# lixinustc/KVQ-Challenge-CVPR-NTIRE2024

Measured on AMD Instinct MI355X. Metric: videos/sec (8-frag x 32 x 224 x 224), higher is better.
Workload: dtype bf16

## Files before the change

include/kvq_hip.h:

```cpp
#ifndef KVQ_HIP_H
#define KVQ_HIP_H

#include <stddef.h>
#include <stdint.h>

#ifdef __cplusplus
extern "C" {
#endif

#define KVQ_ABI_VERSION 31
#define KVQ_MAX_STAGES 4

typedef enum { KVQ_DT_BF16 = 0, KVQ_DT_FP16 = 1 } KvqDtype;

typedef enum {
  KVQ_OK = 0,
  KVQ_ERR_NULL = -1,
  KVQ_ERR_SHAPE = -2,
  KVQ_ERR_UNSUPPORTED = -3,
  KVQ_ERR_WORKSPACE = -4,
  KVQ_ERR_HIP = -5
} KvqStatus;

int kvq_abi_version(void);
// ... 229 lines not shown
int kvq_block_tail(const KvqBlockTailArgs* host_args, void* stream);

int kvq_window_attention(const uint16_t* qkv, const int32_t* tok, const float* rpb, const float* fpb,
                         const float* bias_pack, int table_len, int center, int BW, int nW, int N, int num_heads, int use_mask,
                         int dtype, uint16_t* out, void* stream);

size_t kvq_attn_bias32_bytes(int n_types, int N, int num_heads);
int kvq_attn_bias32_build(const int32_t* tok, const float* rpb, const float* fpb, int table_len, int center,
                          int n_types, int N, int num_heads, int use_mask, void* out, float* max_abs, void* stream);
typedef struct {
  const uint16_t* qkv;
  const void* bias_dense;
  int32_t n_types, BW, nW, N, num_heads, dtype;
  uint16_t* out;
  const uint32_t* tile_skip;
  int32_t dsplit_from;
  const uint16_t* x_ln;
  const uint16_t* w_qkv;
  const float* b_qkv;
  float q_scale;
  const uint32_t* pad_mask;
} KvqAttnDenseArgs;
int kvq_window_attention32(const KvqAttnDenseArgs* host_args, void* stream);

int kvq_patch_im2col(const float* x, int B, int Cin, int T, int H, int W, int pd, int ph, int pw,
                     int dtype, uint16_t* out, void* stream);

int kvq_vqa_head(const float* feat, int B, int L, int C, int64_t stride_b, int64_t stride_l,
                 int64_t stride_c, const float* w1t, const float* w1, const float* b1, int hidden, const float* w2,
                 const float* b2, float* scratch, float* score, void* stream);

int kvq_vqa_head_classes(const float* feat, int B, int L, int C, int64_t stride_b, int64_t stride_l, int64_t stride_c,
                         const float* w1t, const float* b1, int hidden, const float* w2, const float* b2, int num_class,
                         int pre_pool, float* scratch, float* score, void* stream);

int kvq_simple_vqa_head(const float* feat, int B, int T, int Cin, const float* w1, const float* b1,
                        int hidden, const float* w2, const float* b2, float* scratch, float* score,
                        void* stream);

int kvq_fragment_gather(const void* video, int src_is_u8, int C, int T, int H, int W, const int32_t* hoff,
                        const int32_t* woff, int Fh, int Fw, int fs_h, int fs_w, int aligned,
                        const float* host_mean, const float* host_std, float* out, void* stream);
int kvq_fragment_gather_batch(const KvqFragmentSource* src, int C, int T, float* out, void* stream);

int kvq_resize_bilinear(const void* video, int src_is_u8, int C, int T, int H, int W, int rh, int rw, int cy,
                        int cx, int oh, int ow, int round_u8, const float* host_mean, const float* host_std,
// ... 139 lines not shown
```

kvq-challenge-cvpr-ntire2024_amd/_abi.py:

```python
from __future__ import annotations

import ctypes as C
import os
from typing import Optional

from . import _build

MAX_STAGES = 4
K_NAMES = ["im2col", "layernorm", "gemm_qkv", "attn", "gemm_proj", "gemm_fc1", "gemm_fc2", "gemm_merge",
           "gemm_embed", "tail", "embed", "merge"]
K_COUNT = len(K_NAMES)

EPI_BIAS_BF16, EPI_GELU_BF16, EPI_QKV_BF16, EPI_RESID_F32, EPI_STORE_F32, EPI_RELU_BF16, EPI_QGELU_BF16 = range(7)
DT_BF16, DT_FP16 = 0, 1
ABI_VERSION = 31


def dtype_code(dt) -> int:
    import torch
    is_int = isinstance(dt, int) and not isinstance(dt, bool)
    if (is_int and dt == DT_FP16) or (not is_int and dt in (torch.float16, "fp16", "float16")):
        return DT_FP16
    if (is_int and dt == DT_BF16) or (not is_int and dt in (torch.bfloat16, "bf16", "bfloat16")):
        return DT_BF16
# ... 13 lines not shown
                ("num_heads", C.c_int32 * MAX_STAGES), ("window", C.c_int32 * 3), ("mlp_ratio", C.c_int32),
                ("frag_bias", C.c_int32 * MAX_STAGES), ("adaptive_window", C.c_int32 * 3)]


class KvqSwinBlockW(C.Structure):
    _fields_ = [(n, p_void) for n in ("norm1_w", "norm1_b", "rpb_table", "fpb_table", "bias_pack", "qkv_w", "qkv_b", "proj_w",
                                      "proj_b", "norm2_w", "norm2_b", "fc1_w", "fc1_b", "fc2_w", "fc2_b", "tail_pack", "qkv_pack", "bias_dense")]


class KvqSwinMergeW(C.Structure):
    _fields_ = [(n, p_void) for n in ("norm_w", "norm_b", "red_w", "merge_pack")]


class KvqSwinWeights(C.Structure):
    _fields_ = [("embed_w", p_void), ("embed_b", p_void), ("embed_ln_w", p_void), ("embed_ln_b", p_void),
                ("embed_pack", p_void), ("blocks", C.POINTER(KvqSwinBlockW)), ("merges", KvqSwinMergeW * (MAX_STAGES - 1)),
                ("norm_w", p_void), ("norm_b", p_void)]


class KvqAttnDenseArgs(C.Structure):
    _fields_ = [("qkv", p_void), ("bias_dense", p_void), ("n_types", C.c_int32), ("BW", C.c_int32), ("nW", C.c_int32), ("N", C.c_int32),
                ("num_heads", C.c_int32), ("dtype", C.c_int32), ("out", p_void), ("tile_skip", p_void), ("dsplit_from", C.c_int32),
                ("x_ln", p_void), ("w_qkv", p_void), ("b_qkv", p_void), ("q_scale", C.c_float), ("pad_mask", p_void)]


class KvqGemmArgs(C.Structure):
    _fields_ = [("A", p_void), ("W", p_void), ("bias", p_void), ("M", C.c_int32), ("N", C.c_int32),
                ("K", C.c_int32), ("epilogue", C.c_int32), ("out_bf16", p_void), ("out_f32", p_void),
                ("num_heads", C.c_int32), ("q_scale", C.c_float), ("scatter_map", p_void),
                ("map_rows", C.c_int32), ("out_rows", C.c_int32), ("dtype", C.c_int32), ("resid_bf16", p_void), ("resid_f32", p_void),
                ("splitk_ws", p_void), ("splitk_ws_bytes", C.c_size_t), ("ldc", C.c_int32), ("col_off", C.c_int32),
                ("a_gather", p_void), ("a_rows", C.c_int32), ("a_phys_rows", C.c_int32)]


class KvqConvArgs(C.Structure):
    _fields_ = [("x", p_void), ("W", p_void), ("bias", p_void), ("taps", p_void), ("dims5", C.c_int32 * 5),
                ("kernel3", C.c_int32 * 3), ("stride3", C.c_int32 * 3), ("pad3", C.c_int32 * 3), ("Kpad", C.c_int32),
                ("N", C.c_int32), ("epilogue", C.c_int32), ("dtype", C.c_int32), ("out_bf16", p_void), ("out_f32", p_void),
                ("resid_bf16", p_void), ("resid_f32", p_void), ("splitk_ws", p_void), ("splitk_ws_bytes", C.c_size_t),
                ("ldc", C.c_int32), ("col_off", C.c_int32)]


class KvqNetTensor(C.Structure):
    _fields_ = [("B", C.c_int32), ("D", C.c_int32), ("H", C.c_int32), ("W", C.c_int32), ("C", C.c_int32), ("kind", C.c_int32)]


# ... 98 lines not shown
    "kvq_debug_gemm_trace": (i32, [p_void, i32]),
    "kvq_gemm_tile_mode": (i32, [i32]),
    "kvq_patch_embed_supported": (i32, [i32] * 8),
    "kvq_patch_embed_fragments_supported": (i32, [C.POINTER(KvqFragmentSource), i32, i32, i32, i32, i32, i32]),
    "kvq_patch_embed_pack_bytes": (sz, [i32, i32]),
    "kvq_patch_embed_pack": (i32, [p_void, p_void, p_void, p_void, i32, i32, p_void, p_void]),
    "kvq_patch_embed": (i32, [C.POINTER(KvqPatchEmbedArgs), p_void]),
    "kvq_patch_merge_supported": (i32, [i32]),
    "kvq_patch_merge_pack_bytes": (sz, [i32]),
    "kvq_patch_merge_pack": (i32, [p_void, p_void, p_void, i32, i32, p_void, p_void]),
    "kvq_patch_merge": (i32, [C.POINTER(KvqPatchMergeArgs), p_void]),
    "kvq_block_tail_supported": (i32, [i32, i32]),
    "kvq_block_tail_pack_bytes": (sz, [i32, i32]),
    "kvq_block_tail_pack": (i32, [p_void, p_void, p_void, p_void, p_void, p_void, p_void, p_void, i32, i32, p_void,
                                  p_void]),
    "kvq_block_tail_qkv_pack_bytes": (sz, [i32, i32]),
    "kvq_block_tail_qkv_pack": (i32, [p_void, i32, i32, p_void, p_void]),
    "kvq_block_tail": (i32, [C.POINTER(KvqBlockTailArgs), p_void]),
    "kvq_window_attention": (i32, [p_void, p_void, p_void, p_void, p_void, i32, i32, i32, i32, i32, i32, i32, i32, p_void,
                                   p_void]),
    "kvq_attn_bias32_bytes": (sz, [i32, i32, i32]),
    "kvq_attn_bias32_build": (i32, [p_void, p_void, p_void, i32, i32, i32, i32, i32, i32, p_void, p_void, p_void]),
    "kvq_window_attention32": (i32, [C.POINTER(KvqAttnDenseArgs), p_void]),
    "kvq_swin3d_bias_dense_bytes": (sz, [p_void, i32]),
    "kvq_swin3d_bias_dense_build": (i32, [p_void, i32, p_void, p_void, p_void, p_void, p_void]),
    "kvq_patch_im2col": (i32, [p_void, i32, i32, i32, i32, i32, i32, i32, i32, i32, p_void, p_void]),
    "kvq_vqa_head": (i32, [p_void, i32, i32, i32, i64, i64, i64, p_void, p_void, p_void, i32, p_void, p_void, p_void,
                           p_void, p_void]),
    "kvq_vqa_head_classes": (i32, [p_void, i32, i32, i32, i64, i64, i64, p_void, p_void, i32, p_void, p_void, i32, i32, p_void,
                                   p_void, p_void]),
    "kvq_simple_vqa_head": (i32, [p_void, i32, i32, i32, p_void, p_void, i32, p_void, p_void, p_void, p_void,
                                  p_void]),
    "kvq_resize_bilinear": (i32, [p_void, i32, i32, i32, i32, i32, i32, i32, i32, i32, i32, i32, i32, C.POINTER(f32),
                                  C.POINTER(f32), p_void, p_void]),
    "kvq_upsample_frames_out_dims": (i32, [i32, i32, C.c_double, C.POINTER(i32 * 2)]),
    "kvq_upsample_frames": (i32, [p_void, i32, i32, i32, i32, i32, C.c_double, p_void, p_void]),
    "kvq_im2col_nd": (i32, [p_void, i32, i32, C.POINTER(i64 * 5), C.POINTER(i32 * 5), C.POINTER(i32 * 3),
                            C.POINTER(i32 * 3), C.POINTER(i32 * 3), i32, p_void, p_void]),
    "kvq_pack_channels_last8": (i32, [p_void, C.POINTER(i32 * 5), C.POINTER(i64 * 5), i32, p_void, p_void]),
    "kvq_conv_stem_direct": (i32, [p_void, C.POINTER(i32 * 5), p_void, p_void, i32, C.POINTER(i32 * 3), C.POINTER(i32 * 3),
                                   C.POINTER(i32 * 3), i32, i32, p_void, p_void]),
    "kvq_pack_clip_cl4": (i32, [p_void, C.POINTER(i32 * 5), i32, i32, p_void, p_void]),
    "kvq_conv_stem_pool": (i32, [p_void, C.POINTER(i32 * 5), p_void, p_void, i32, i32, i32, p_void, p_void]),
    "kvq_conv_stem64_pool": (i32, [p_void, C.POINTER(i32 * 5), p_void, i32, p_void, p_void, i32, i32, p_void, i32, i32, p_void]),
    "kvq_slow_bottleneck_pack_bytes": (C.c_size_t, [i32, i32, i32]),
    "kvq_slow_bottleneck": (i32, [p_void, C.POINTER(i32 * 4), i32, i32, i32, p_void, i32, p_void, i32, p_void]),
# ... 76 lines not shown
```

kvq-challenge-cvpr-ntire2024_amd/csrc/attn32.hip:

```cpp
#include <stdlib.h>

#include "common.hpp"

#ifndef A32_ABL
#define A32_ABL 0
#endif
#ifndef A32_SUM
#define A32_SUM 0
#endif
#if (A32_ABL & 2)
#define A32_EXP(x) ((x) * 0.001f + 1.0f)
#else
#define A32_EXP(x) __builtin_amdgcn_exp2f(x)
#endif

#ifdef KVQ_DIAG
#define A32_DIAG_FLAG(x) (x)
#else
#define A32_DIAG_FLAG(x) false
#endif

namespace kvq {

constexpr int A32_KB = 13;
// ... 196 lines not shown
  }
  ls += ls1;
  if (A32_SUM == 1) ls = (lv0[0] + lv0[1]) + (lv1[0] + lv1[1]);
  ls = a32_pair_sum(ls);
  a32_finish<E>(O, ls, orow, store);
#undef A32_NR
}

struct Attn32Params {
  const uint16_t* qkv;
  const u32x4* image;
  int BW, nW, N, nH, n_types, qsplit;
  uint16_t* out;
  const uint32_t* tile_skip;
  int dsplit_from;
  const uint16_t* x_ln;
  const uint16_t* w_qkv;
  const float* b_qkv;
  float q_scale;
  uint16_t* q_out;
  const uint32_t* pad_mask;
  bool no_q_store;
  bool image_one;
};

template <typename E, int KS>
__device__ __forceinline__ void a32_fused_qkv(const Attn32Params& p, unsigned char* slot, int bw, int h, int N) {
  using V8 = typename E::v8;
  const int tid = threadIdx.x, lane = tid & 63, j = lane & 15, g = lane >> 4;
  const int wave = __builtin_amdgcn_readfirstlane(tid >> 6);
  const int C = KS * 32;
  const size_t Mtot = (size_t)p.BW * N;
  const uint16_t* xw = p.x_ln + (size_t)bw * N * C;
  uint16_t* qo = p.q_out + ((size_t)h * Mtot + (size_t)bw * N) * 32;
  V8 wf[6][KS];
  float bias[6][4];
#pragma unroll
  for (int c = 0; c < 6; ++c) {
    const int which = c >> 1, half = c & 1, frow = which * C + h * 32 + half * 16;
#pragma unroll
    for (int ks = 0; ks < KS; ++ks) wf[c][ks] = *reinterpret_cast<const V8*>(p.w_qkv + (size_t)(frow + j) * C + 32 * ks + 8 * g);
    const f32x4 b4 = *reinterpret_cast<const f32x4*>(p.b_qkv + frow + 4 * g);
#pragma unroll
    for (int r = 0; r < 4; ++r) bias[c][r] = b4[r];
  }
  const int nrt = (N + 15) / 16;
  V8 xn[KS];
  {
    const int rowc = min(16 * wave + j, N - 1);
#pragma unroll
    for (int ks = 0; ks < KS; ++ks) xn[ks] = *reinterpret_cast<const V8*>(xw + (size_t)rowc * C + 32 * ks + 8 * g);
  }
#pragma unroll 1
  for (int rt = wave; rt < nrt; rt += A32_WAVES) {
    const int row = 16 * rt + j;
    V8 xf[KS];
#pragma unroll
    for (int ks = 0; ks < KS; ++ks) xf[ks] = xn[ks];
    if (rt + A32_WAVES < nrt) {
      const int rowc = min(row + 16 * A32_WAVES, N - 1);
#pragma unroll
      for (int ks = 0; ks < KS; ++ks) xn[ks] = *reinterpret_cast<const V8*>(xw + (size_t)rowc * C + 32 * ks + 8 * g);
    }
#pragma unroll
    for (int c = 0; c < 6; ++c) {
      const int which = c >> 1, half = c & 1;
      f32x4 acc = {0.f, 0.f, 0.f, 0.f};
#pragma unroll
      for (int ks = 0; ks < KS; ++ks) acc = E::mfma16(wf[c][ks], xf[ks], acc);
      const float sc = which == 0 ? p.q_scale : 1.f;
      const u32x2 v = {E::pack2((acc[0] + bias[c][0]) * sc, (acc[1] + bias[c][1]) * sc),
                       E::pack2((acc[2] + bias[c][2]) * sc, (acc[3] + bias[c][3]) * sc)};
      if (row < N) {
        if (which == 0) {
          if (!A32_DIAG_FLAG(p.no_q_store)) *reinterpret_cast<u32x2*>(qo + (size_t)row * 32 + half * 16 + 4 * g) = v;
        } else if (which == 1) {
          *reinterpret_cast<u32x2*>(slot + row * 64 + (((2 * half + (g >> 1)) ^ ((row >> 2) & 3)) << 4) + (g & 1) * 8) = v;
        } else {
          *reinterpret_cast<u32x2*>(slot + A32_K_BYTES + row * 64 + (16 * half + 4 * g) * 2) = v;
        }
      }
    }
  }
}

template <typename E, bool FUSED, bool DSPLIT, bool SHORT = false>
__global__ __launch_bounds__(A32_WAVES * 64, 3) __attribute__((amdgpu_waves_per_eu(3, 3))) void window_attention32_kernel(Attn32Params p) {
  fp16_saturate_mode();
  extern __shared__ __attribute__((aligned(16))) unsigned char smem[];
  int* ticket = reinterpret_cast<int*>(smem + A32_OFF_CTR);
  using V8 = typename E::v8;
  const int nclip = p.BW / p.nW, nrep = p.nW / p.n_types, npair = p.n_types * p.nH, per_pair = nclip * nrep * p.qsplit;
  const int xcd = blockIdx.x & 7, slot_i = blockIdx.x >> 3;
  int pair, clip, rep, part;
  if (FUSED) {
    const int per_type = p.nH * nclip * nrep, wt_ = (slot_i / per_type) * 8 + xcd, sub = slot_i % per_type;
    if (wt_ >= p.n_types) return;
    const int h_ = sub % p.nH, rest = sub / p.nH;
    pair = wt_ * p.nH + h_; clip = rest % nclip; rep = rest / nclip; part = 0;
  } else {
    const int sub = slot_i % per_pair;
    pair = (slot_i / per_pair) * 8 + xcd;
    clip = sub % nclip; rep = (sub / nclip) % nrep; part = sub / (nclip * nrep);
  }
  if (pair >= npair) return;
  const int wt = pair / p.nH, h = pair - wt * p.nH, w = rep * p.n_types + wt, bw = clip * p.nW + w;
  const int tid = threadIdx.x, lane = tid & 63, N = p.N, nqb = (N + 31) >> 5;
  const int wave = __builtin_amdgcn_readfirstlane(tid >> 6);
  const size_t Mtot = (size_t)p.BW * N;
  const int C = p.nH * 32;
  const uint16_t* Qg = p.qkv + ((size_t)h * Mtot + (size_t)bw * N) * 32;

  if (tid < 64) *reinterpret_cast<u32x4*>(smem + A32_OFF_ZERO + tid * 16) = (u32x4){0u, 0u, 0u, 0u};
  if (FUSED) {
    for (int i = tid; i < (A32_ROWS - N) * 8; i += A32_WAVES * 64)
      *reinterpret_cast<u32x4*>(smem + (i & 4 ? A32_K_BYTES : 0) + (N + (i >> 3)) * 64 + (i & 3) * 16) = (u32x4){0u, 0u, 0u, 0u};
    a32_fused_qkv<E, 3>(p, smem, bw, h, N);
  } else {
    const uint16_t* Kg = p.qkv + ((size_t)(1 * p.nH + h) * Mtot + (size_t)bw * N) * 32;
    const uint16_t* Vg = p.qkv + ((size_t)(2 * p.nH + h) * Mtot + (size_t)bw * N) * 32;
    const __amdgpu_buffer_rsrc_t rk = __builtin_amdgcn_make_buffer_rsrc(const_cast<uint16_t*>(Kg), 0, N * 64, 0x00020000);
    const __amdgpu_buffer_rsrc_t rv = __builtin_amdgcn_make_buffer_rsrc(const_cast<uint16_t*>(Vg), 0, N * 64, 0x00020000);
    const unsigned vo_k = (unsigned)(lane >> 2) * 64u + (unsigned)((lane & 3) ^ ((lane >> 4) & 3)) * 16u, vo_v = (unsigned)lane * 16u;
    for (int it = wave; it < A32_ROWS / 16; it += A32_WAVES) {
      __builtin_amdgcn_raw_ptr_buffer_load_lds(rk, (a32_lds_t)(smem + it * 1024), 16, vo_k, it * 1024, 0, 0);
      __builtin_amdgcn_raw_ptr_buffer_load_lds(rv, (a32_lds_t)(smem + A32_K_BYTES + it * 1024), 16, vo_v, it * 1024, 0, 0);
    }
  }
  const int q_lo = part * nqb / p.qsplit, q_hi = (part + 1) * nqb / p.qsplit;
  if (tid == 0) *ticket = q_lo;
  asm volatile("s_waitcnt vmcnt(0)" ::: "memory");
  __syncthreads();
  if (!FUSED && p.pad_mask) {
    const uint32_t* pm = p.pad_mask + (size_t)w * A32_KB;
    const int c = tid & 3;
    const float* kb = p.b_qkv + C + h * 32 + 8 * c;
    const float* vb = p.b_qkv + 2 * C + h * 32 + 8 * c;
    const u32x4 kc = {E::pack2(kb[0], kb[1]), E::pack2(kb[2], kb[3]), E::pack2(kb[4], kb[5]), E::pack2(kb[6], kb[7])};
    const u32x4 vc = {E::pack2(vb[0], vb[1]), E::pack2(vb[2], vb[3]), E::pack2(vb[4], vb[5]), E::pack2(vb[6], vb[7])};
    for (int r = tid >> 2; r < N; r += A32_WAVES * 16)
// ... 106 lines not shown
    const int half = tile & 1, blk = tile >> 1, qb = blk / A32_KB, kb = blk - qb * A32_KB, qq = 32 * qb + ql;
    const int2 tq = tokL[qq < N ? qq : N - 1];
    const float shift = rmax[qq < N ? qq : N - 1];
    float v[8];
#pragma unroll
    for (int e = 0; e < 8; ++e) {
      const int r = 8 * half + e, key = 32 * kb + (r & 3) + 8 * (r >> 2) + 4 * hi;
      float b = 0.f;
      if (key >= N) {
        b = A32_OFF;
      } else if (qq < N) {
        bool masked;
        b = value(tq, key, &masked);
        if (masked) b = -100.0f;
        b -= shift;
      }
      v[e] = b;
    }
    *reinterpret_cast<u32x4*>(img + (size_t)tile * 512 + lane * 8) =
        (u32x4){Fp16::pack2_raw(v[0], v[1]), Fp16::pack2_raw(v[2], v[3]), Fp16::pack2_raw(v[4], v[5]), Fp16::pack2_raw(v[6], v[7])};
  }
}

template <typename E, bool FUSED, bool DSPLIT, bool SHORT>
static int launch_attn32_form(const Attn32Params& p, hipStream_t st) {
  auto kern = window_attention32_kernel<E, FUSED, DSPLIT, SHORT>;
  LdsOptIn opt;
  if (int rc = opt.ensure(reinterpret_cast<const void*>(kern), A32_LDS)) return rc;
  const int nclip = p.BW / p.nW, nrep = p.nW / p.n_types, npair = p.n_types * p.nH;
  unsigned grid = (unsigned)(8 * ceil_div(npair, 8) * nclip * nrep * p.qsplit);
  if (FUSED) grid = (unsigned)(8 * ceil_div(p.n_types, 8) * p.nH * nclip * nrep);
  hipLaunchKernelGGL(kern, dim3(grid), dim3(A32_WAVES * 64), A32_LDS, st, p);
  KVQ_CHECK_LAUNCH("window_attention32_kernel");
  return KVQ_OK;
}

template <typename E, bool FUSED, bool DSPLIT>
static int launch_attn32(const Attn32Params& p, hipStream_t st) {
  return p.N > 384 && p.N <= 392 ? launch_attn32_form<E, FUSED, DSPLIT, true>(p, st) : launch_attn32_form<E, FUSED, DSPLIT, false>(p, st);
}

template <typename E>
static int launch_attn32_e(const Attn32Params& p, hipStream_t st) {
  if (p.x_ln) return p.dsplit_from >= 0 ? launch_attn32<E, true, true>(p, st) : launch_attn32<E, true, false>(p, st);
  return p.dsplit_from >= 0 ? launch_attn32<E, false, true>(p, st) : launch_attn32<E, false, false>(p, st);
}

}

extern "C" size_t kvq_attn_bias32_bytes(int n_types, int N, int num_heads) {
  if (n_types <= 0 || N < 1 || N > 400 || num_heads <= 0) return 0;
  return (size_t)n_types * num_heads * ((N + 31) / 32) * kvq::A32_KB * 2048 + 2048;
}

extern "C" int kvq_attn_bias32_build(const int32_t* tok, const float* rpb, const float* fpb, int table_len, int center,
                                          int nW, int N, int num_heads, int use_mask, void* out, float* max_abs, void* stream) {
  using namespace kvq;
  KVQ_REQUIRE(tok && rpb && out, KVQ_ERR_NULL, "kvq_attn_bias32_build: NULL pointer");
  KVQ_REQUIRE(kvq_attn_bias32_bytes(nW, N, num_heads) > 0 && table_len > 0, KVQ_ERR_SHAPE,
              "kvq_attn_bias32_build: bad shape nW=%d N=%d nH=%d", nW, N, num_heads);
  KVQ_REQUIRE(((size_t)out & 15) == 0, KVQ_ERR_SHAPE, "kvq_attn_bias32_build: out must be 16-byte aligned");
  Bias32BuildParams p{tok, rpb, fpb, table_len, center, nW, N, num_heads, use_mask, (uint16_t*)out, (unsigned*)max_abs};
  const size_t lds = (size_t)table_len * 8 + (size_t)N * 12;
  KVQ_REQUIRE(lds <= 64 * 1024, KVQ_ERR_UNSUPPORTED, "kvq_attn_bias32_build: table of %d entries does not fit the builder's LDS", table_len);
  hipLaunchKernelGGL(bias32_build_kernel, dim3((unsigned)num_heads, (unsigned)nW), dim3(256), lds, (hipStream_t)stream, p);
  KVQ_CHECK_LAUNCH("bias32_build_kernel");
  return KVQ_OK;
}

extern "C" int kvq_window_attention32(const KvqAttnDenseArgs* a, void* stream) {
  using namespace kvq;
  KVQ_REQUIRE(a && a->qkv && a->bias_dense && a->out, KVQ_ERR_NULL, "kvq_window_attention32: NULL pointer");
  const int BW = a->BW, nW = a->nW, N = a->N, num_heads = a->num_heads, n_types = a->n_types;
  KVQ_REQUIRE(BW > 0 && nW > 0 && BW % nW == 0 && num_heads > 0 && n_types > 0 && nW % n_types == 0, KVQ_ERR_SHAPE,
              "kvq_window_attention32: bad shape BW=%d nW=%d n_types=%d nH=%d", BW, nW, n_types, num_heads);
  KVQ_REQUIRE(N >= 1 && N <= 400, KVQ_ERR_UNSUPPORTED, "kvq_window_attention32: window of %d tokens unsupported (1..400)", N);
  KVQ_REQUIRE(((size_t)a->bias_dense & 15) == 0, KVQ_ERR_SHAPE, "kvq_window_attention32: the bias image must be 16-byte aligned");
  KVQ_REQUIRE(a->dtype == KVQ_DT_BF16 || a->dtype == KVQ_DT_FP16, KVQ_ERR_UNSUPPORTED, "kvq_window_attention32: dtype %d", a->dtype);
  KVQ_REQUIRE(a->dsplit_from < 0 || (N == 392 && a->dsplit_from < nW), KVQ_ERR_UNSUPPORTED,
              "kvq_window_attention32: depth-split windows need the (8,7,7) window (N = 392); got N=%d from=%d", N, a->dsplit_from);
  const int units = BW * num_heads, nqb = (N + 31) / 32;
  int qsplit = units >= 768 ? 1 : 768 / units;
  const int qsplit_max = latency_mode() ? 4 : 1;
  qsplit = qsplit > qsplit_max ? qsplit_max : qsplit;
  qsplit = qsplit > nqb ? nqb : qsplit;
  Attn32Params p{a->qkv, (const u32x4*)a->bias_dense, BW, nW, N, num_heads, n_types, qsplit, a->out, a->tile_skip,
                     a->dsplit_from < 0 ? -1 : a->dsplit_from};
#ifdef KVQ_DIAG
  { static const bool one = getenv("KVQ_IMAGE_ONE_TYPE") && atoi(getenv("KVQ_IMAGE_ONE_TYPE")) == 1; p.image_one = one; }
  { static const bool nq = getenv("KVQ_NO_Q_STORE") && atoi(getenv("KVQ_NO_Q_STORE")) == 1; p.no_q_store = nq; }
#endif
  if (a->pad_mask) {
    KVQ_REQUIRE(a->b_qkv && !a->x_ln, KVQ_ERR_NULL, "kvq_window_attention32: pad_mask needs b_qkv (and excludes the fused projection)");
    p.pad_mask = a->pad_mask; p.b_qkv = a->b_qkv;
  }
  if (a->x_ln) {
    const int C = 32 * num_heads;
    KVQ_REQUIRE(a->w_qkv && a->b_qkv, KVQ_ERR_NULL, "kvq_window_attention32: x_ln without w_qkv / b_qkv");
    KVQ_REQUIRE(C == 96, KVQ_ERR_UNSUPPORTED, "kvq_window_attention32: the fused qkv projection is built for C = 96 (got %d)", C);
    KVQ_REQUIRE((((size_t)a->x_ln | (size_t)a->w_qkv | (size_t)a->b_qkv) & 15) == 0, KVQ_ERR_SHAPE,
                "kvq_window_attention32: x_ln / w_qkv / b_qkv must be 16-byte aligned");
    p.qsplit = 1;
    p.x_ln = a->x_ln; p.w_qkv = a->w_qkv; p.b_qkv = a->b_qkv; p.q_scale = a->q_scale; p.q_out = const_cast<uint16_t*>(a->qkv);
  }
  hipStream_t st = (hipStream_t)stream;
  return a->dtype == KVQ_DT_FP16 ? launch_attn32_e<Fp16>(p, st) : launch_attn32_e<Bf16>(p, st);
}
```

kvq-challenge-cvpr-ntire2024_amd/csrc/plan.hip:

```cpp
#include <math.h>
#include <stdlib.h>
#include <string.h>

#include <vector>

#include "common.hpp"
#include "tail.hpp"

#ifdef KVQ_DIAG
static int skip_mask() {
  static const int m = [] {
    const int v = getenv("KVQ_SKIP") ? atoi(getenv("KVQ_SKIP")) : 0;
    if (v) fprintf(stderr, "libkvq_hip (KVQ_DIAG build): KVQ_SKIP=%d leaves launch families out - scores are GARBAGE, timing only\n", v);
    return v;
  }();
  return m;
}
#else
static constexpr int skip_mask() { return 0; }
#endif

namespace kvq {

struct StageGeom {
// ... 425 lines not shown
  const bool embed_fused = w->embed_pack && kvq_patch_embed_supported(cfg.in_chans, cfg.patch[0], cfg.patch[1], cfg.patch[2], cfg.embed_dim, pl->T, pl->H, pl->W);
  auto fused_tail = [&](int i, int bk) -> bool { return w->blocks[bk].tail_pack && kvq_block_tail_supported(pl->st[i].C, cfg.mlp_ratio * pl->st[i].C); };
  auto attn_fuses_qkv = [&](int i, int bk) -> bool {
    const StageGeom& g = pl->st[i];
    const KvqSwinBlockW& bw = w->blocks[bk];
    return bw.bias_dense && bw.qkv_b && g.Lp == g.L && g.C == 96 && g.N <= 400;
  };
  bool x16[KVQ_MAX_STAGES] = {false, false, false, false};
  if (resid16_on && !any_tap) {
    int blk0 = 0;
    for (int i = 0; i < cfg.num_stages - 1 && i <= stage_hi; blk0 += pl->st[i].depth, ++i) {
      if (i < stage_lo) continue;
      const StageGeom& g = pl->st[i];
      const bool produced16 = i == 0 ? (stage_lo == 0 && embed_fused) : (i > stage_lo && (fused_merge(i - 1) || pl->dtype == KVQ_DT_FP16));
      bool ok = produced16;
      for (int b = 0; ok && b < g.depth; ++b) {
        const KvqSwinBlockW& bw = w->blocks[blk0 + b];
        const int par = (b & 1) && g.shifted_any ? 1 : 0;
        ok = fused_tail(i, blk0 + b) && bw.norm1_w && bw.norm1_b && g.d_dst[par];
      }
      x16[i] = ok;
    }
  }
  bool x16_cur = false;
  auto f32_only = [&](const char* what) -> int {
    KVQ_REQUIRE(!x16_cur, KVQ_ERR_UNSUPPORTED, "kvq_swin3d_forward: internal: %s on an fp16 residual stream", what);
    return KVQ_OK;
  };

  const int L0 = pl->D0 * pl->H0 * pl->W0, E = cfg.embed_dim;
  float* cur = xa;
  float* oth = xb;
  bool first_ln1_ready = false;
  if (stage_lo > 0) {
    const StageGeom& g0 = pl->st[stage_lo];
    KVQ_CHECK_HIP(hipMemcpyAsync(xa, io, (size_t)B * g0.L * g0.C * sizeof(float), hipMemcpyDeviceToDevice, st));
  } else if (embed_fused) {
    KvqPatchEmbedArgs ea{};
    ea.x = x; ea.frag = frag; ea.B = B; ea.in_chans = cfg.in_chans; ea.T = pl->T; ea.H = pl->H; ea.W = pl->W;
    ea.pd = cfg.patch[0]; ea.ph = cfg.patch[1]; ea.pw = cfg.patch[2]; ea.embed_dim = E; ea.pack = w->embed_pack;
    ea.has_norm = w->embed_ln_w ? 1 : 0; ea.out = xa; ea.eps = 1e-5f; ea.dtype = pl->dtype; ea.out_f16 = x16[0] ? 1 : 0;
    x16_cur = x16[0];
    const StageGeom& g0 = pl->st[0];
    if (g0.Lp == g0.L && g0.d_dst[0] && w->blocks[0].norm1_w && w->blocks[0].norm1_b) {
      ea.next_norm_w = w->blocks[0].norm1_w; ea.next_norm_b = w->blocks[0].norm1_b; ea.next_dst = g0.d_dst[0];
      ea.next_ln = bln; ea.next_rows = g0.Lp;
// ... 25 lines not shown
    KVQ_CHECK_HIP(hipMemcpyAsync(pl->taps[idx], cur, elems * sizeof(float), hipMemcpyDeviceToDevice, st));
    return KVQ_OK;
  };
  if (stage_lo == 0) KVQ_TRY(tap(0, (size_t)B * L0 * E));

  int blk = 0;
  for (int i = 0; i < stage_lo; ++i) blk += pl->st[i].depth;
  size_t out_elems = 0;
  bool merged_ln1_ready = false;
  for (int i = stage_lo; i <= stage_hi; ++i) {
    const StageGeom& g = pl->st[i];
    const int C = g.C, M = B * g.Lp, ML = B * g.L;
    bool ln1_ready = (i == 0 && first_ln1_ready) || merged_ln1_ready;
    bool qkv_ready = false;
    merged_ln1_ready = false;
    if (i == stage_lo && i > 0) cur = xa, oth = xb;
    for (int b = 0; b < g.depth; ++b, ++blk) {
      const KvqSwinBlockW& bw = w->blocks[blk];
      KVQ_REQUIRE(bw.norm1_w && bw.rpb_table && bw.qkv_w && bw.proj_w && bw.fc1_w && bw.fc2_w, KVQ_ERR_NULL,
                  "kvq_swin3d_forward: block %d weights incomplete", blk);
      const int par = (b & 1) && g.shifted_any ? 1 : 0;
      const bool fuse_qkv = attn_fuses_qkv(i, blk);
      const float qs = bw.bias_dense ? kQScaleLog2 : kQScale;
      if (g.Lp != g.L && bw.qkv_b && qkv_ready) {
      } else if (g.Lp != g.L && bw.qkv_b) {
        if (!ln1_ready) KVQ_TRY(ln(pl, st, cur, nullptr, 1, g.L, g.L, C, bw.norm1_w, bw.norm1_b, bln, nullptr, x16_cur));
        KVQ_TRY(gemm(pl, st, KVQ_K_GEMM_QKV, bln, bw.qkv_w, bw.qkv_b, ML, 3 * C, C, KVQ_EPI_QKV_BF16, bbig, nullptr, g.nH,
                     qs, g.d_dst[par], g.L, g.Lp));
        if (!(bw.bias_dense && g.d_padmask[par]))
          KVQ_TRY(kvq_qkv_fill_pad(bbig, bw.qkv_b, g.d_pad[par], g.Lp - g.L, B, g.Lp, g.nH, qs, pl->dtype, st));
      } else if (!qkv_ready) {
        if (!ln1_ready) KVQ_TRY(ln(pl, st, cur, g.d_src[par], 1, g.L, g.Lp, C, bw.norm1_w, bw.norm1_b, bln, nullptr, x16_cur));
        if (!fuse_qkv)
          KVQ_TRY_UNLESS(8 | (i == cfg.num_stages - 1 ? 32 : 0), gemm(pl, st, KVQ_K_GEMM_QKV, bln, bw.qkv_w, bw.qkv_b, M, 3 * C, C, KVQ_EPI_QKV_BF16, bbig, nullptr, g.nH, qs));
      }
      ln1_ready = false;
      qkv_ready = false;
      if (bw.bias_dense) {
        Bracket br(pl, st, KVQ_K_ATTN, 4 + par, 4.0 * M * g.N * C + (fuse_qkv ? 6.0 * M * C * C : 0.0),
                   (fuse_qkv ? 2.0 * 2.0 * M * C + 6.0 * C * C : 2.0 * 4.0 * M * C) + (double)kvq_swin3d_bias_dense_bytes(pl, blk));
        KvqAttnDenseArgs aa{};
        aa.qkv = bbig; aa.bias_dense = bw.bias_dense; aa.n_types = bias_types(g, par); aa.BW = B * g.nW; aa.nW = g.nW; aa.N = g.N;
        aa.num_heads = g.nH; aa.dtype = pl->dtype; aa.out = bo; aa.tile_skip = (const uint32_t*)g.d_skip[par];
        const int slabs = g.Dp / g.ws[0];
        aa.dsplit_from = (par == 1 && g.N == 392 && g.ws[0] == 8 && g.ws[1] == 7 && g.ws[2] == 7 && g.ss[0] == 4 && slabs >= 1)
                             ? g.nW - g.nW / slabs : -1;
        if (fuse_qkv) { aa.x_ln = bln; aa.w_qkv = bw.qkv_w; aa.b_qkv = bw.qkv_b; aa.q_scale = qs; }
        if (g.Lp != g.L && bw.qkv_b && g.d_padmask[par]) { aa.pad_mask = (const uint32_t*)g.d_padmask[par]; aa.b_qkv = bw.qkv_b; }
        KVQ_TRY_UNLESS(1 | (i == cfg.num_stages - 1 ? 32 : 0), kvq_window_attention32(&aa, st));
      } else {
        Bracket br(pl, st, KVQ_K_ATTN, (cfg.frag_bias[i] ? 2 : 0) + par, 4.0 * M * g.N * C, 2.0 * 4.0 * M * C);
        KVQ_TRY(kvq_window_attention(bbig, g.d_tok[par], bw.rpb_table, cfg.frag_bias[i] ? bw.fpb_table : nullptr,
                                     bw.bias_pack,
                                     pl->table_len, pl->center, B * g.nW, g.nW, g.N, g.nH, par, pl->dtype, bo,
                                     st));
      }
      const int hidden = cfg.mlp_ratio * C;
      if (fused_tail(i, blk)) {
        KvqBlockTailArgs ta{};
        ta.attn = bo; ta.x = cur; ta.scatter_map = g.d_src[par]; ta.map_rows = g.Lp; ta.out_rows = g.L;
        ta.M = M; ta.C = C; ta.hidden = hidden; ta.pack = bw.tail_pack; ta.eps = 1e-5f; ta.dtype = pl->dtype;
        ta.x_f16 = x16_cur ? 1 : 0;
        const int npar = ((b + 1) & 1) && g.shifted_any ? 1 : 0;
        if (g.Lp != g.L) ta.attn_gather = g.d_dst[par];
        const bool padded_qkv = g.Lp != g.L && b + 1 < g.depth && g.d_dst[npar] && g.d_padmask[npar] && w->blocks[blk + 1].bias_dense;
        const int32_t* nmap = (g.Lp == g.L || padded_qkv) ? g.d_dst[npar] : nullptr;
        if (b + 1 < g.depth && nmap) {
          const KvqSwinBlockW& nb = w->blocks[blk + 1];
          KVQ_REQUIRE(nb.norm1_w && nb.norm1_b, KVQ_ERR_NULL, "kvq_swin3d_forward: block %d norm1 missing", blk + 1);
          ta.next_norm_w = nb.norm1_w; ta.next_norm_b = nb.norm1_b; ta.next_dst = nmap;
          ta.next_rows = g.Lp;
          if (!attn_fuses_qkv(i, blk + 1) && nb.qkv_pack && nb.qkv_b && nb.bias_dense && (g.Lp == g.L || padded_qkv) && kvq_block_tail_qkv_pack_bytes(C, hidden) > 0) {
            ta.next_qkv_pack = nb.qkv_pack; ta.next_qkv_b = nb.qkv_b; ta.qkv_out = bbig; ta.q_scale = kQScaleLog2; ta.num_heads = g.nH;
            qkv_ready = true;
          } else if (g.Lp == g.L) {
            ta.next_ln = bln;
            ln1_ready = true;
          } else {
            ta.next_norm_w = nullptr; ta.next_norm_b = nullptr; ta.next_dst = nullptr; ta.next_rows = 0;
          }
        }
        Bracket br(pl, st, KVQ_K_TAIL, kvq::tailmm_geometry_code(C, hidden) * 1000 + (C / 32) * 10 + (ln1_ready ? 1 : 0) + (qkv_ready ? 2 : 0), 2.0 * M * C * C + 4.0 * (double)ML * C * hidden + (qkv_ready ? 6.0 * M * C * C : 0.0),
                   (double)M * C * 2.0 + (double)ML * C * ((x16_cur ? 4.0 : 8.0) + (ln1_ready ? 2.0 : 0.0) + (qkv_ready ? 6.0 : 0.0)));
        KVQ_TRY_UNLESS(C <= 192 ? 2 : 4, kvq_block_tail(&ta, st));
        continue;
      }
      KVQ_TRY(f32_only("the proj / MLP GEMM chain"));
      if (g.Lp != g.L) {
        KvqGemmArgs pa{};
        pa.A = bo; pa.W = bw.proj_w; pa.bias = bw.proj_b; pa.M = ML; pa.N = C; pa.K = C; pa.epilogue = KVQ_EPI_RESID_F32; pa.out_f32 = cur;
        pa.dtype = pl->dtype; pa.a_gather = g.d_dst[par]; pa.a_rows = g.L; pa.a_phys_rows = g.Lp;
        Bracket br(pl, st, KVQ_K_GEMM_PROJ, gemm_variant(ML, C, C) * 10 + KVQ_EPI_RESID_F32, 2.0 * M * C * C,
                   2.0 * ((double)ML * C + (double)C * C) + 8.0 * ML * C);
        KVQ_TRY(kvq_gemm_bf16(&pa, st));
      } else {
        KVQ_TRY_UNLESS(i == cfg.num_stages - 1 ? 32 : 0, gemm(pl, st, KVQ_K_GEMM_PROJ, bo, bw.proj_w, bw.proj_b, M, C, C, KVQ_EPI_RESID_F32, nullptr, cur, 0, 1.f,
                     g.d_src[par], g.Lp, g.L));
// ... 74 lines not shown
```

kvq-challenge-cvpr-ntire2024_amd/kernels.py:

```python
from __future__ import annotations

import ctypes as C
from typing import Optional, Sequence

import torch

from . import _abi
from ._abi import check, current_stream, dtype_code, lib, ptr, stream_of

HALF_TYPES = (torch.float16, torch.bfloat16)


def _need_gpu(*ts):
    for t in ts:
        if t is not None and not t.is_cuda:
            raise _abi.KvqError("kvq_amd kernels need tensors on a HIP device (no CPU fallback exists)")


def device_name() -> str:
    buf = C.create_string_buffer(256)
    check(lib().kvq_device_name(buf, 256), "kvq_device_name")
    return buf.value.decode()


# ... 79 lines not shown
    check(lib().kvq_window_attention(ptr(qkv), ptr(tok), ptr(rpb), ptr(fpb), ptr(bias_pack), rpb.shape[0], center, BW, nW, N, nH,
                                     int(use_mask), dtype_code(qkv.dtype), ptr(out), current_stream()),
          "kvq_window_attention")
    return out


LOG2E = 1.4426950408889634


def attn_bias32(tok: torch.Tensor, rpb: torch.Tensor, fpb: Optional[torch.Tensor], center: int, nW: int, N: int, use_mask: bool):
    _need_gpu(tok, rpb, fpb)
    nH = rpb.shape[1]
    out = torch.empty(lib().kvq_attn_bias32_bytes(nW, N, nH), dtype=torch.uint8, device=rpb.device)
    big = torch.zeros(1, dtype=torch.float32, device=rpb.device)
    check(lib().kvq_attn_bias32_build(ptr(tok), ptr(rpb), ptr(fpb), rpb.shape[0], center, nW, N, nH, int(use_mask),
                                      ptr(out), ptr(big), current_stream()), "kvq_attn_bias32_build")
    out.max_abs_bias = big
    return out


def window_attention32(qkv: torch.Tensor, image: torch.Tensor, nW: int, N: int, n_types: Optional[int] = None,
                       tile_skip: Optional[torch.Tensor] = None, out: Optional[torch.Tensor] = None, dsplit_from: int = -1,
                       x_ln: Optional[torch.Tensor] = None, w_qkv: Optional[torch.Tensor] = None, b_qkv: Optional[torch.Tensor] = None,
                       q_scale: float = 1.0, pad_mask: Optional[torch.Tensor] = None):
    _need_gpu(qkv, image, tile_skip, out, pad_mask)
    assert qkv.dtype in HALF_TYPES and qkv.is_contiguous()
    nH = qkv.shape[1]
    BW = qkv.shape[2] // N
    if out is None:
        out = torch.empty(BW * N, nH * 32, dtype=qkv.dtype, device=qkv.device)
    a = _abi.KvqAttnDenseArgs()
    a.qkv, a.bias_dense, a.n_types, a.BW, a.nW, a.N, a.num_heads = ptr(qkv), ptr(image), nW if n_types is None else n_types, BW, nW, N, nH
    a.dtype, a.out, a.tile_skip, a.dsplit_from = dtype_code(qkv.dtype), ptr(out), ptr(tile_skip), dsplit_from
    if x_ln is not None:
        _need_gpu(x_ln, w_qkv, b_qkv)
        assert x_ln.dtype == qkv.dtype == w_qkv.dtype and x_ln.is_contiguous() and w_qkv.is_contiguous() and b_qkv.dtype == torch.float32
        a.x_ln, a.w_qkv, a.b_qkv, a.q_scale = ptr(x_ln), ptr(w_qkv), ptr(b_qkv), q_scale
    if pad_mask is not None:
        _need_gpu(b_qkv)
        assert pad_mask.dtype == torch.int32 and pad_mask.is_contiguous() and (b_qkv is None or b_qkv.dtype == torch.float32)
        a.pad_mask, a.b_qkv = ptr(pad_mask), ptr(b_qkv)
    check(lib().kvq_window_attention32(C.byref(a), current_stream()), "kvq_window_attention32")
    return out


def patch_im2col(x: torch.Tensor, patch: Sequence[int], out_dtype=torch.float16):
    _need_gpu(x)
    assert x.dtype == torch.float32 and x.is_contiguous()
    B, Cin, T, H, W = x.shape
    pd, ph, pw = patch
    D, Hh, Ww = -(-T // pd), -(-H // ph), -(-W // pw)
    out = torch.empty(B * D * Hh * Ww, Cin * pd * ph * pw, dtype=out_dtype, device=x.device)
    check(lib().kvq_patch_im2col(ptr(x), B, Cin, T, H, W, pd, ph, pw, dtype_code(out_dtype), ptr(out),
                                 current_stream()), "kvq_patch_im2col")
    return out


def vqa_head(feat: torch.Tensor, w1, b1, w2, b2, w1t=None):
    _need_gpu(feat, w1, b1, w2, b2, w1t)
    assert feat.dtype == torch.float32 and feat.dim() == 5
    B, Cc, D, H, W = feat.shape
    L = D * H * W
    sb, sc, sd, sh, sw = feat.stride()
    if not (sh == W * sw and sd == H * sh):
# ... 727 lines not shown
```

Measured before the change: 364.7.

## Fuse norm1 LayerNorm and window gather into fused-QKV attention kernel

Adds a NORM variant of the fused-QKV window attention kernel. It reads the fp16 residual stream directly through the window map, applies LayerNorm with gamma and beta staged in LDS, and then runs the QKV projection. The planner uses it when it is eligible, skipping the separate LN launch and the LN that the previous block tail produced, which removes a write and read of the normalized activations. The cost is more per-row work and extra LDS inside the attention kernel, plus gathered, non-contiguous row loads.

After: 366.1 (median of 6 runs). About the same (+0.4%).

```diff
diff --git a/include/kvq_hip.h b/include/kvq_hip.h
--- a/include/kvq_hip.h
+++ b/include/kvq_hip.h
@@ -275,6 +275,15 @@
   const uint32_t* pad_mask;
 } KvqAttnDenseArgs;
 int kvq_window_attention32(const KvqAttnDenseArgs* host_args, void* stream);
+typedef struct KvqAttnNorm1Args {
+  const void* x;
+  const int32_t* window_map;
+  int L;
+  const float* norm1_w;
+  const float* norm1_b;
+  float eps;
+} KvqAttnNorm1Args;
+int kvq_window_attention32_norm1(const KvqAttnDenseArgs* host_args, const KvqAttnNorm1Args* norm, void* stream);
 
 int kvq_patch_im2col(const float* x, int B, int Cin, int T, int H, int W, int pd, int ph, int pw,
                      int dtype, uint16_t* out, void* stream);
diff --git a/kvq-challenge-cvpr-ntire2024_amd/_abi.py b/kvq-challenge-cvpr-ntire2024_amd/_abi.py
--- a/kvq-challenge-cvpr-ntire2024_amd/_abi.py
+++ b/kvq-challenge-cvpr-ntire2024_amd/_abi.py
@@ -59,6 +59,10 @@
     _fields_ = [("qkv", p_void), ("bias_dense", p_void), ("n_types", C.c_int32), ("BW", C.c_int32), ("nW", C.c_int32), ("N", C.c_int32),
                 ("num_heads", C.c_int32), ("dtype", C.c_int32), ("out", p_void), ("tile_skip", p_void), ("dsplit_from", C.c_int32),
                 ("x_ln", p_void), ("w_qkv", p_void), ("b_qkv", p_void), ("q_scale", C.c_float), ("pad_mask", p_void)]
+
+
+class KvqAttnNorm1Args(C.Structure):
+    _fields_ = [("x", p_void), ("window_map", p_void), ("L", C.c_int32), ("norm1_w", p_void), ("norm1_b", p_void), ("eps", C.c_float)]
 
 
 class KvqGemmArgs(C.Structure):
@@ -203,6 +207,7 @@
     "kvq_attn_bias32_bytes": (sz, [i32, i32, i32]),
     "kvq_attn_bias32_build": (i32, [p_void, p_void, p_void, i32, i32, i32, i32, i32, i32, p_void, p_void, p_void]),
     "kvq_window_attention32": (i32, [C.POINTER(KvqAttnDenseArgs), p_void]),
+    "kvq_window_attention32_norm1": (i32, [C.POINTER(KvqAttnDenseArgs), C.POINTER(KvqAttnNorm1Args), p_void]),
     "kvq_swin3d_bias_dense_bytes": (sz, [p_void, i32]),
     "kvq_swin3d_bias_dense_build": (i32, [p_void, i32, p_void, p_void, p_void, p_void, p_void]),
     "kvq_patch_im2col": (i32, [p_void, i32, i32, i32, i32, i32, i32, i32, i32, i32, p_void, p_void]),
diff --git a/kvq-challenge-cvpr-ntire2024_amd/csrc/attn32.hip b/kvq-challenge-cvpr-ntire2024_amd/csrc/attn32.hip
--- a/kvq-challenge-cvpr-ntire2024_amd/csrc/attn32.hip
+++ b/kvq-challenge-cvpr-ntire2024_amd/csrc/attn32.hip
@@ -242,16 +242,29 @@
   const uint32_t* pad_mask;
   bool no_q_store;
   bool image_one;
+  const uint16_t* x16;
+  const int32_t* map;
+  int L;
+  const float* n1w;
+  const float* n1b;
+  float eps;
 };
-
-template <typename E, int KS>
+constexpr int A32_OFF_NRM = A32_LDS;
+constexpr int A32_LDS_NORM = A32_OFF_NRM + 2 * 96 * 4;
+
+template <typename E, int KS, bool NORM = false>
 __device__ __forceinline__ void a32_fused_qkv(const Attn32Params& p, unsigned char* slot, int bw, int h, int N) {
   using V8 = typename E::v8;
   const int tid = threadIdx.x, lane = tid & 63, j = lane & 15, g = lane >> 4;
   const int wave = __builtin_amdgcn_readfirstlane(tid >> 6);
   const int C = KS * 32;
   const size_t Mtot = (size_t)p.BW * N;
-  const uint16_t* xw = p.x_ln + (size_t)bw * N * C;
+  const uint16_t* xw = NORM ? nullptr : p.x_ln + (size_t)bw * N * C;
+  const int clip = NORM ? bw / p.nW : 0, wl = NORM ? bw - clip * p.nW : 0;
+  auto rowp = [&](int r) __attribute__((always_inline)) -> const uint16_t* {
+    if constexpr (NORM) return p.x16 + ((size_t)clip * p.L + p.map[(size_t)wl * N + r]) * C;
+    else return xw + (size_t)r * C;
+  };
   uint16_t* qo = p.q_out + ((size_t)h * Mtot + (size_t)bw * N) * 32;
   V8 wf[6][KS];
   float bias[6][4];
@@ -269,7 +282,7 @@
   {
     const int rowc = min(16 * wave + j, N - 1);
 #pragma unroll
-    for (int ks = 0; ks < KS; ++ks) xn[ks] = *reinterpret_cast<const V8*>(xw + (size_t)rowc * C + 32 * ks + 8 * g);
+    for (int ks = 0; ks < KS; ++ks) xn[ks] = *reinterpret_cast<const V8*>(rowp(rowc) + 32 * ks + 8 * g);
   }
 #pragma unroll 1
   for (int rt = wave; rt < nrt; rt += A32_WAVES) {
@@ -280,7 +293,46 @@
     if (rt + A32_WAVES < nrt) {
       const int rowc = min(row + 16 * A32_WAVES, N - 1);
 #pragma unroll
-      for (int ks = 0; ks < KS; ++ks) xn[ks] = *reinterpret_cast<const V8*>(xw + (size_t)rowc * C + 32 * ks + 8 * g);
+      for (int ks = 0; ks < KS; ++ks) xn[ks] = *reinterpret_cast<const V8*>(rowp(rowc) + 32 * ks + 8 * g);
+    }
+    if constexpr (NORM) {
+      typedef __attribute__((ext_vector_type(8))) _Float16 h8;
+      const float* nrm = reinterpret_cast<const float*>(slot + A32_OFF_NRM);
+      float s = 0.f;
+#pragma unroll
+      for (int ks = 0; ks < KS; ++ks) {
+        const h8 v = __builtin_bit_cast(h8, xf[ks]);
+        s += ((float)v[0] + (float)v[1]) + ((float)v[2] + (float)v[3]) + (((float)v[4] + (float)v[5]) + ((float)v[6] + (float)v[7]));
+      }
+      s += __shfl_xor(s, 16);
+      s += __shfl_xor(s, 32);
+      const float mean = s / (float)C;
+      float sq = 0.f;
+#pragma unroll
+      for (int ks = 0; ks < KS; ++ks) {
+        const h8 v = __builtin_bit_cast(h8, xf[ks]);
+#pragma unroll
+        for (int e = 0; e < 8; ++e) {
+          const float d = (float)v[e] - mean;
+          sq += d * d;
+        }
+      }
+      sq += __shfl_xor(sq, 16);
+      sq += __shfl_xor(sq, 32);
+      const float rstd = rsqrtf(sq / (float)C + p.eps), nmr = -mean * rstd;
+#pragma unroll
+      for (int ks = 0; ks < KS; ++ks) {
+        const h8 v = __builtin_bit_cast(h8, xf[ks]);
+        const f32x4 g0 = *reinterpret_cast<const f32x4*>(nrm + 32 * ks + 8 * g), g1 = *reinterpret_cast<const f32x4*>(nrm + 32 * ks + 8 * g + 4);
+        const f32x4 b0 = *reinterpret_cast<const f32x4*>(nrm + C + 32 * ks + 8 * g), b1 = *reinterpret_cast<const f32x4*>(nrm + C + 32 * ks + 8 * g + 4);
+        float y[8];
+#pragma unroll
+        for (int e = 0; e < 4; ++e) {
+          y[e] = fmaf(fmaf((float)v[e], rstd, nmr), g0[e], b0[e]);
+          y[4 + e] = fmaf(fmaf((float)v[4 + e], rstd, nmr), g1[e], b1[e]);
+        }
+        xf[ks] = __builtin_bit_cast(V8, (u32x4){E::pack2(y[0], y[1]), E::pack2(y[2], y[3]), E::pack2(y[4], y[5]), E::pack2(y[6], y[7])});
+      }
     }
 #pragma unroll
     for (int c = 0; c < 6; ++c) {
@@ -304,7 +356,7 @@
   }
 }
 
-template <typename E, bool FUSED, bool DSPLIT, bool SHORT = false>
+template <typename E, bool FUSED, bool DSPLIT, bool SHORT = false, bool NORM = false>
 __global__ __launch_bounds__(A32_WAVES * 64, 3) __attribute__((amdgpu_waves_per_eu(3, 3))) void window_attention32_kernel(Attn32Params p) {
   fp16_saturate_mode();
   extern __shared__ __attribute__((aligned(16))) unsigned char smem[];
@@ -335,7 +387,11 @@
   if (FUSED) {
     for (int i = tid; i < (A32_ROWS - N) * 8; i += A32_WAVES * 64)
       *reinterpret_cast<u32x4*>(smem + (i & 4 ? A32_K_BYTES : 0) + (N + (i >> 3)) * 64 + (i & 3) * 16) = (u32x4){0u, 0u, 0u, 0u};
-    a32_fused_qkv<E, 3>(p, smem, bw, h, N);
+    if constexpr (NORM) {
+      if (tid < 2 * 96) reinterpret_cast<float*>(smem + A32_OFF_NRM)[tid] = tid < 96 ? p.n1w[tid] : p.n1b[tid - 96];
+      __syncthreads();
+    }
+    a32_fused_qkv<E, 3, NORM>(p, smem, bw, h, N);
   } else {
     const uint16_t* Kg = p.qkv + ((size_t)(1 * p.nH + h) * Mtot + (size_t)bw * N) * 32;
     const uint16_t* Vg = p.qkv + ((size_t)(2 * p.nH + h) * Mtot + (size_t)bw * N) * 32;
@@ -488,15 +544,16 @@
   }
 }
 
-template <typename E, bool FUSED, bool DSPLIT, bool SHORT>
+template <typename E, bool FUSED, bool DSPLIT, bool SHORT, bool NORM = false>
 static int launch_attn32_form(const Attn32Params& p, hipStream_t st) {
-  auto kern = window_attention32_kernel<E, FUSED, DSPLIT, SHORT>;
+  auto kern = window_attention32_kernel<E, FUSED, DSPLIT, SHORT, NORM>;
+  constexpr int lds = NORM ? A32_LDS_NORM : A32_LDS;
   LdsOptIn opt;
-  if (int rc = opt.ensure(reinterpret_cast<const void*>(kern), A32_LDS)) return rc;
+  if (int rc = opt.ensure(reinterpret_cast<const void*>(kern), lds)) return rc;
   const int nclip = p.BW / p.nW, nrep = p.nW / p.n_types, npair = p.n_types * p.nH;
   unsigned grid = (unsigned)(8 * ceil_div(npair, 8) * nclip * nrep * p.qsplit);
   if (FUSED) grid = (unsigned)(8 * ceil_div(p.n_types, 8) * p.nH * nclip * nrep);
-  hipLaunchKernelGGL(kern, dim3(grid), dim3(A32_WAVES * 64), A32_LDS, st, p);
+  hipLaunchKernelGGL(kern, dim3(grid), dim3(A32_WAVES * 64), lds, st, p);
   KVQ_CHECK_LAUNCH("window_attention32_kernel");
   return KVQ_OK;
 }
@@ -506,8 +563,14 @@
   return p.N > 384 && p.N <= 392 ? launch_attn32_form<E, FUSED, DSPLIT, true>(p, st) : launch_attn32_form<E, FUSED, DSPLIT, false>(p, st);
 }
 
+template <typename E, bool DSPLIT>
+static int launch_attn32_norm(const Attn32Params& p, hipStream_t st) {
+  return p.N > 384 && p.N <= 392 ? launch_attn32_form<E, true, DSPLIT, true, true>(p, st) : launch_attn32_form<E, true, DSPLIT, false, true>(p, st);
+}
+
 template <typename E>
 static int launch_attn32_e(const Attn32Params& p, hipStream_t st) {
+  if (p.x16) return p.dsplit_from >= 0 ? launch_attn32_norm<E, true>(p, st) : launch_attn32_norm<E, false>(p, st);
   if (p.x_ln) return p.dsplit_from >= 0 ? launch_attn32<E, true, true>(p, st) : launch_attn32<E, true, false>(p, st);
   return p.dsplit_from >= 0 ? launch_attn32<E, false, true>(p, st) : launch_attn32<E, false, false>(p, st);
 }
@@ -534,7 +597,7 @@
   return KVQ_OK;
 }
 
-extern "C" int kvq_window_attention32(const KvqAttnDenseArgs* a, void* stream) {
+static int attn32_entry(const KvqAttnDenseArgs* a, const KvqAttnNorm1Args* n, void* stream) {
   using namespace kvq;
   KVQ_REQUIRE(a && a->qkv && a->bias_dense && a->out, KVQ_ERR_NULL, "kvq_window_attention32: NULL pointer");
   const int BW = a->BW, nW = a->nW, N = a->N, num_heads = a->num_heads, n_types = a->n_types;
@@ -560,15 +623,29 @@
     KVQ_REQUIRE(a->b_qkv && !a->x_ln, KVQ_ERR_NULL, "kvq_window_attention32: pad_mask needs b_qkv (and excludes the fused projection)");
     p.pad_mask = a->pad_mask; p.b_qkv = a->b_qkv;
   }
-  if (a->x_ln) {
+  if (n) {
+    KVQ_REQUIRE(n->x && n->window_map && n->norm1_w && n->norm1_b && !a->x_ln && !a->pad_mask, KVQ_ERR_NULL,
+                "kvq_window_attention32_norm1: NULL pointer, or x_ln / pad_mask given");
+    KVQ_REQUIRE(n->L == nW * N, KVQ_ERR_SHAPE, "kvq_window_attention32_norm1: un-padded partitions only (L=%d, nW=%d, N=%d)", n->L, nW, N);
+    KVQ_REQUIRE(((size_t)n->x & 15) == 0, KVQ_ERR_SHAPE, "kvq_window_attention32_norm1: x must be 16-byte aligned");
+    p.x16 = (const uint16_t*)n->x; p.map = n->window_map; p.L = n->L; p.n1w = n->norm1_w; p.n1b = n->norm1_b; p.eps = n->eps;
+  }
+  if (a->x_ln || n) {
     const int C = 32 * num_heads;
     KVQ_REQUIRE(a->w_qkv && a->b_qkv, KVQ_ERR_NULL, "kvq_window_attention32: x_ln without w_qkv / b_qkv");
     KVQ_REQUIRE(C == 96, KVQ_ERR_UNSUPPORTED, "kvq_window_attention32: the fused qkv projection is built for C = 96 (got %d)", C);
     KVQ_REQUIRE((((size_t)a->x_ln | (size_t)a->w_qkv | (size_t)a->b_qkv) & 15) == 0, KVQ_ERR_SHAPE,
                 "kvq_window_attention32: x_ln / w_qkv / b_qkv must be 16-byte aligned");
     p.qsplit = 1;
-    p.x_ln = a->x_ln; p.w_qkv = a->w_qkv; p.b_qkv = a->b_qkv; p.q_scale = a->q_scale; p.q_out = const_cast<uint16_t*>(a->qkv);
+    p.x_ln = (const uint16_t*)a->x_ln; p.w_qkv = a->w_qkv; p.b_qkv = a->b_qkv; p.q_scale = a->q_scale; p.q_out = const_cast<uint16_t*>(a->qkv);
   }
   hipStream_t st = (hipStream_t)stream;
   return a->dtype == KVQ_DT_FP16 ? launch_attn32_e<Fp16>(p, st) : launch_attn32_e<Bf16>(p, st);
 }
+
+extern "C" int kvq_window_attention32(const KvqAttnDenseArgs* a, void* stream) { return attn32_entry(a, nullptr, stream); }
+
+extern "C" int kvq_window_attention32_norm1(const KvqAttnDenseArgs* a, const KvqAttnNorm1Args* n, void* stream) {
+  KVQ_REQUIRE(n, KVQ_ERR_NULL, "kvq_window_attention32_norm1: NULL norm1 arguments");
+  return attn32_entry(a, n, stream);
+}
diff --git a/kvq-challenge-cvpr-ntire2024_amd/csrc/plan.hip b/kvq-challenge-cvpr-ntire2024_amd/csrc/plan.hip
--- a/kvq-challenge-cvpr-ntire2024_amd/csrc/plan.hip
+++ b/kvq-challenge-cvpr-ntire2024_amd/csrc/plan.hip
@@ -471,6 +471,15 @@
       x16[i] = ok;
     }
   }
+  auto attn_norms = [&](int i, int bk) -> bool {
+#ifdef KVQ_NO_ATTN_NORM1
+    return false;
+#else
+    const StageGeom& g = pl->st[i];
+    const KvqSwinBlockW& bw = w->blocks[bk];
+    return x16[i] && attn_fuses_qkv(i, bk) && bw.norm1_w && bw.norm1_b && g.d_src[0] && (!g.shifted_any || g.d_src[1]);
+#endif
+  };
   bool x16_cur = false;
   auto f32_only = [&](const char* what) -> int {
     KVQ_REQUIRE(!x16_cur, KVQ_ERR_UNSUPPORTED, "kvq_swin3d_forward: internal: %s on an fp16 residual stream", what);
@@ -542,6 +551,7 @@
       const int par = (b & 1) && g.shifted_any ? 1 : 0;
       const bool fuse_qkv = attn_fuses_qkv(i, blk);
       const float qs = bw.bias_dense ? kQScaleLog2 : kQScale;
+      const bool norm_in_attn = fuse_qkv && !ln1_ready && !qkv_ready && attn_norms(i, blk);
       if (g.Lp != g.L && bw.qkv_b && qkv_ready) {
       } else if (g.Lp != g.L && bw.qkv_b) {
         if (!ln1_ready) KVQ_TRY(ln(pl, st, cur, nullptr, 1, g.L, g.L, C, bw.norm1_w, bw.norm1_b, bln, nullptr, x16_cur));
@@ -550,14 +560,14 @@
         if (!(bw.bias_dense && g.d_padmask[par]))
           KVQ_TRY(kvq_qkv_fill_pad(bbig, bw.qkv_b, g.d_pad[par], g.Lp - g.L, B, g.Lp, g.nH, qs, pl->dtype, st));
       } else if (!qkv_ready) {
-        if (!ln1_ready) KVQ_TRY(ln(pl, st, cur, g.d_src[par], 1, g.L, g.Lp, C, bw.norm1_w, bw.norm1_b, bln, nullptr, x16_cur));
+        if (!ln1_ready && !norm_in_attn) KVQ_TRY(ln(pl, st, cur, g.d_src[par], 1, g.L, g.Lp, C, bw.norm1_w, bw.norm1_b, bln, nullptr, x16_cur));
         if (!fuse_qkv)
           KVQ_TRY_UNLESS(8 | (i == cfg.num_stages - 1 ? 32 : 0), gemm(pl, st, KVQ_K_GEMM_QKV, bln, bw.qkv_w, bw.qkv_b, M, 3 * C, C, KVQ_EPI_QKV_BF16, bbig, nullptr, g.nH, qs));
       }
       ln1_ready = false;
       qkv_ready = false;
       if (bw.bias_dense) {
-        Bracket br(pl, st, KVQ_K_ATTN, 4 + par, 4.0 * M * g.N * C + (fuse_qkv ? 6.0 * M * C * C : 0.0),
+        Bracket br(pl, st, KVQ_K_ATTN, (norm_in_attn ? 6 : 4) + par, 4.0 * M * g.N * C + (fuse_qkv ? 6.0 * M * C * C : 0.0),
                    (fuse_qkv ? 2.0 * 2.0 * M * C + 6.0 * C * C : 2.0 * 4.0 * M * C) + (double)kvq_swin3d_bias_dense_bytes(pl, blk));
         KvqAttnDenseArgs aa{};
         aa.qkv = bbig; aa.bias_dense = bw.bias_dense; aa.n_types = bias_types(g, par); aa.BW = B * g.nW; aa.nW = g.nW; aa.N = g.N;
@@ -565,9 +575,15 @@
         const int slabs = g.Dp / g.ws[0];
         aa.dsplit_from = (par == 1 && g.N == 392 && g.ws[0] == 8 && g.ws[1] == 7 && g.ws[2] == 7 && g.ss[0] == 4 && slabs >= 1)
                              ? g.nW - g.nW / slabs : -1;
-        if (fuse_qkv) { aa.x_ln = bln; aa.w_qkv = bw.qkv_w; aa.b_qkv = bw.qkv_b; aa.q_scale = qs; }
+        if (fuse_qkv) { aa.x_ln = norm_in_attn ? nullptr : bln; aa.w_qkv = bw.qkv_w; aa.b_qkv = bw.qkv_b; aa.q_scale = qs; }
         if (g.Lp != g.L && bw.qkv_b && g.d_padmask[par]) { aa.pad_mask = (const uint32_t*)g.d_padmask[par]; aa.b_qkv = bw.qkv_b; }
-        KVQ_TRY_UNLESS(1 | (i == cfg.num_stages - 1 ? 32 : 0), kvq_window_attention32(&aa, st));
+        if (norm_in_attn) {
+          KvqAttnNorm1Args na{};
+          na.x = cur; na.window_map = g.d_src[par]; na.L = g.L; na.norm1_w = bw.norm1_w; na.norm1_b = bw.norm1_b; na.eps = 1e-5f;
+          KVQ_TRY_UNLESS(1, kvq_window_attention32_norm1(&aa, &na, st));
+        } else {
+          KVQ_TRY_UNLESS(1 | (i == cfg.num_stages - 1 ? 32 : 0), kvq_window_attention32(&aa, st));
+        }
       } else {
         Bracket br(pl, st, KVQ_K_ATTN, (cfg.frag_bias[i] ? 2 : 0) + par, 4.0 * M * g.N * C, 2.0 * 4.0 * M * C);
         KVQ_TRY(kvq_window_attention(bbig, g.d_tok[par], bw.rpb_table, cfg.frag_bias[i] ? bw.fpb_table : nullptr,
@@ -593,6 +609,8 @@
           if (!attn_fuses_qkv(i, blk + 1) && nb.qkv_pack && nb.qkv_b && nb.bias_dense && (g.Lp == g.L || padded_qkv) && kvq_block_tail_qkv_pack_bytes(C, hidden) > 0) {
             ta.next_qkv_pack = nb.qkv_pack; ta.next_qkv_b = nb.qkv_b; ta.qkv_out = bbig; ta.q_scale = kQScaleLog2; ta.num_heads = g.nH;
             qkv_ready = true;
+          } else if (g.Lp == g.L && attn_norms(i, blk + 1)) {
+            ta.next_norm_w = nullptr; ta.next_norm_b = nullptr; ta.next_dst = nullptr; ta.next_rows = 0;
           } else if (g.Lp == g.L) {
             ta.next_ln = bln;
             ln1_ready = true;
diff --git a/kvq-challenge-cvpr-ntire2024_amd/kernels.py b/kvq-challenge-cvpr-ntire2024_amd/kernels.py
--- a/kvq-challenge-cvpr-ntire2024_amd/kernels.py
+++ b/kvq-challenge-cvpr-ntire2024_amd/kernels.py
@@ -125,7 +125,8 @@
 def window_attention32(qkv: torch.Tensor, image: torch.Tensor, nW: int, N: int, n_types: Optional[int] = None,
                        tile_skip: Optional[torch.Tensor] = None, out: Optional[torch.Tensor] = None, dsplit_from: int = -1,
                        x_ln: Optional[torch.Tensor] = None, w_qkv: Optional[torch.Tensor] = None, b_qkv: Optional[torch.Tensor] = None,
-                       q_scale: float = 1.0, pad_mask: Optional[torch.Tensor] = None):
+                       q_scale: float = 1.0, pad_mask: Optional[torch.Tensor] = None, x16: Optional[torch.Tensor] = None,
+                       window_map: Optional[torch.Tensor] = None, norm1=None, eps: float = 1e-5):
     _need_gpu(qkv, image, tile_skip, out, pad_mask)
     assert qkv.dtype in HALF_TYPES and qkv.is_contiguous()
     nH = qkv.shape[1]
@@ -143,6 +144,14 @@
         _need_gpu(b_qkv)
         assert pad_mask.dtype == torch.int32 and pad_mask.is_contiguous() and (b_qkv is None or b_qkv.dtype == torch.float32)
         a.pad_mask, a.b_qkv = ptr(pad_mask), ptr(b_qkv)
+    if x16 is not None:
+        _need_gpu(x16, window_map, w_qkv, b_qkv, *norm1)
+        assert x_ln is None and x16.dtype == torch.float16 and x16.is_contiguous() and window_map.dtype == torch.int32
+        a.w_qkv, a.b_qkv, a.q_scale = ptr(w_qkv), ptr(b_qkv), q_scale
+        n = _abi.KvqAttnNorm1Args()
+        n.x, n.window_map, n.L, n.norm1_w, n.norm1_b, n.eps = ptr(x16), ptr(window_map), nW * N, ptr(norm1[0]), ptr(norm1[1]), eps
+        check(lib().kvq_window_attention32_norm1(C.byref(a), C.byref(n), current_stream()), "kvq_window_attention32_norm1")
+        return out
     check(lib().kvq_window_attention32(C.byref(a), current_stream()), "kvq_window_attention32")
     return out
 
```
